# jinmang2/anomaly_detection_on_video

Hardware: AMD Instinct MI355X
Metric: 16-frame 224² RGB clips/sec (I3D extract→MIL score), 1/2/4/8 GPU + %MFMA-peak (higher is better)
Workload: dtype f32

## Files before the change

### anomaly_detection_on_video_amd/_lib.py

```python
from __future__ import annotations

import ctypes as C
import os
from typing import Optional

import torch

_HERE = os.path.dirname(os.path.abspath(__file__))
LIB_PATH = os.path.join(_HERE, "csrc", "libadvhip.so")

ALGO_AUTO = 0
ALGO_IGEMM_128x128 = 1
ALGO_IGEMM_128x64 = 2
ALGO_IGEMM_64x64 = 3
ALGO_IGEMM_64x128 = 4
ALGO_IGEMM_128x128x32 = 5
ALGO_IGEMM_128x64x32 = 6
ALGO_IGEMM_64x64x32 = 7
ALGO_IGEMM_64x128x32 = 8
ALGO_IGEMM_256x64 = 9
ALGO_FAST_BASE = 32
IGEMM_ALGOS = (1, 2, 3, 4, 5, 6, 7, 8)
FAST_ALGOS = tuple(ALGO_FAST_BASE + a for a in IGEMM_ALGOS)
ALGO_DMA_BASE = 64
DMA_ALGOS = tuple(ALGO_DMA_BASE + a for a in (1, 2, 3, 4, 6, 7, 8))
ALGO_DMA4_BASE = 96
DMA4_ALGOS = tuple(ALGO_DMA4_BASE + a for a in (2, 3, 4))
ALGO_BF16X3_BASE = 128
BF16X3_ALGOS = tuple(ALGO_BF16X3_BASE + a for a in (5, 6))
ALGO_DMA2_BASE = 160
DMA2_ALGOS = tuple(ALGO_DMA2_BASE + a for a in (1, 2, 3, 4, 6, 7, 8, 9))
ALGO_TSPAN_128x64 = 192
ALGO_MIXED_128x64 = 200
ALGO_PERSIST_BASE = 224
PERSIST_ALGOS = tuple(ALGO_PERSIST_BASE + t + 8 * (w - 1) for w in (1, 2, 3) for t in (2, 3))


def algo_tile(algo: int):
    if algo in (ALGO_TSPAN_128x64, ALGO_MIXED_128x64):
        return (128, 64, 16)
    if ALGO_PERSIST_BASE <= algo < ALGO_PERSIST_BASE + 32:
        return (128 if (algo - ALGO_PERSIST_BASE) & 7 == 2 else 64, 64, 16)
    if algo == ALGO_DMA2_BASE + ALGO_IGEMM_256x64:
        return (256, 64, 16)
    if algo >= ALGO_DMA2_BASE:
        algo -= ALGO_DMA2_BASE
    if algo >= ALGO_BF16X3_BASE:
        algo -= ALGO_BF16X3_BASE
    if algo >= ALGO_DMA4_BASE:
        algo -= ALGO_DMA4_BASE
    if algo >= ALGO_DMA_BASE:
        algo -= ALGO_DMA_BASE
    if algo >= ALGO_FAST_BASE:
        algo -= ALGO_FAST_BASE
    t = (algo - 1) & 3
    return (128 if t in (0, 1) else 64, 128 if t in (0, 3) else 64, 32 if algo >= 5 else 16)


class HipExtensionError(RuntimeError):
    pass


class ConvDesc(C.Structure):
    _fields_ = [(n, C.c_int32) for n in (
        "B", "Cin", "T", "H", "W", "Cout", "kt", "kh", "kw", "st", "sh", "sw", "pt", "ph", "pw",
        "relu", "algo", "splits")]


_P = C.c_void_p
_I = C.c_int32
_L = C.c_int64
# ... 2 lines not shown
class ConvEpilogue(C.Structure):
    _fields_ = ([(n, C.c_void_p) for n in ("y_preact", "dact_z", "ln_u", "ln_mu", "ln_rs", "splitk_counters")] + [("splitk_counter_bytes", C.c_int64)]
                + [("avgpool_out", C.c_void_p)])


class ColsumItem(C.Structure):
    _fields_ = [("src", C.c_void_p), ("dst", C.c_void_p), ("rows", C.c_int64), ("cols", C.c_int32), ("period", C.c_int32)]


class AdamItem(C.Structure):
    _fields_ = [(n, C.c_void_p) for n in ("param", "grad", "exp_avg", "exp_avg_sq", "step")] + [("n", C.c_int64)]


class NtItem(C.Structure):
    _fields_ = [(n, C.c_void_p) for n in ("A", "B", "C", "rowsum")] + [("M", C.c_int32), ("N", C.c_int32), ("lda", C.c_int64), ("ldb", C.c_int64)]


class GemmDesc(C.Structure):
    _fields_ = ([(n, C.c_int32) for n in ("M", "N", "K", "batch")]
                + [(n, C.c_int64) for n in ("sAb", "sAm", "sAk", "sBb", "sBk", "sBn", "sCb", "sCm", "sCn")]
                + [("alpha", C.c_float), ("beta", C.c_float), ("act", C.c_int32)]
                + [(n, C.c_void_p) for n in ("bias_m", "bias_n", "ln_u", "ln_mu", "ln_rs", "residual")])


SIGNATURES = {
    "advhip_abi_version": (C.c_int, []),
    "advhip_last_error": (C.c_char_p, []),
    "advhip_target_arch": (C.c_char_p, []),
    "advhip_conv3d_out_dims": (C.c_int, [C.POINTER(ConvDesc), C.POINTER(_I), C.POINTER(_I), C.POINTER(_I)]),
    "advhip_conv3d_packed_rows": (C.c_int, [C.POINTER(ConvDesc)]),
    "advhip_conv3d_pack_weight_f32": (C.c_int, [C.POINTER(ConvDesc), _P, _P, _P]),
    "advhip_conv3d_pack_weight_bf16x3": (C.c_int, [C.POINTER(ConvDesc), _P, _P, _P]),
    "advhip_conv3d_build_ktab": (C.c_int, [C.POINTER(ConvDesc), _P, _P]),
    "advhip_bn_fold_f32": (C.c_int, [_P, _P, _P, _P, C.c_float, _I, _P, _P, _P]),
    "advhip_conv3d_workspace_bytes": (_L, [C.POINTER(ConvDesc)]),
    "advhip_conv3d_bn_act_f32": (C.c_int, [C.POINTER(ConvDesc), _P, _P, _P, _P, _P, _P, _P, _P, _L, _P]),
    "advhip_conv3d_bn_act_strided_f32": (C.c_int, [C.POINTER(ConvDesc), _P, _L, _P, _P, _P, _P, _P, _P, _L, _P, _L, _P]),
    "advhip_conv3d_pool_out_dims": (C.c_int, [C.POINTER(ConvDesc)] + [_I] * 6 + [C.POINTER(_I)] * 3),
    "advhip_conv3d_relu_maxpool233_workspace_bytes": (_L, [C.POINTER(ConvDesc)]),
    "advhip_conv3d_bn_relu_maxpool233_f32": (C.c_int, [C.POINTER(ConvDesc), _P, _L, _P, _P, _P, _P, _P, _L, _P, _L, _P]),
    "advhip_split_w_plane_floats": (_I, [_I]),
    "advhip_split_w_f32": (C.c_int, [_P, _P, _L, _I, _P]),
    "advhip_conv3d_s2w_build_ktab": (C.c_int, [C.POINTER(ConvDesc), _P, _P]),
    "advhip_conv3d_s2w_bn_relu_maxpool233_f32": (C.c_int, [C.POINTER(ConvDesc), _P, _L, _P, _P, _P, _P, _P, _L, _P, _L, _P]),
    "advhip_conv3d_u8_table_sizes": (C.c_int, [C.POINTER(ConvDesc), C.POINTER(C.c_int64), C.POINTER(C.c_int64)]),
    "advhip_conv3d_u8_build_tables": (C.c_int, [C.POINTER(ConvDesc), _I, _I, _P, C.c_float, _P, _P, _P]),
    "advhip_conv3d_u8_taps_table_sizes": (C.c_int, [C.POINTER(ConvDesc), C.POINTER(C.c_int64), C.POINTER(C.c_int64), C.POINTER(C.c_int64)]),
    "advhip_conv3d_u8_taps_build_tables": (C.c_int, [C.POINTER(ConvDesc), _I, _I, _P, C.c_float, _P, _P, _P, _P]),
    "advhip_conv3d_u8_taps_tencrop_bn_relu_maxpool233_f32": (C.c_int, [C.POINTER(ConvDesc), _P, _L, _I, _I, _L, _L, _P, _P, _P, _P, _P,
                                                                       C.c_float, _P, _L, _P, _L, _P]),
    "advhip_conv3d_u8_tencrop_bn_relu_maxpool233_f32": (C.c_int, [C.POINTER(ConvDesc), _P, _L, _I, _I, _L, _P, _P, _P, _P, _P,
                                                                  C.c_float, _P, _L, _P, _L, _P]),
    "advhip_conv3d_u8_taps_tencrop_bn_relu_maxpool233_strided_f32": (C.c_int, [C.POINTER(ConvDesc), _P, _L, _I, _I, _I, _L, _L, _P, _P, _P, _P, _P,
                                                                               C.c_float, _P, _L, _P, _L, _P]),
    "advhip_conv3d_u8_tencrop_bn_relu_maxpool233_strided_f32": (C.c_int, [C.POINTER(ConvDesc), _P, _L, _I, _I, _I, _L, _P, _P, _P, _P, _P,
                                                                          C.c_float, _P, _L, _P, _L, _P]),
    "advhip_conv3d_bn_act_maxpool211_f32": (C.c_int, [C.POINTER(ConvDesc), _P, _L, _P, _P, _P, _P, _P, _P, _L, _P]),
    "advhip_bgemm_f32": (C.c_int, [C.POINTER(GemmDesc), _P, _P, _P, _P]),
    "advhip_gemm_nt_f32": (C.c_int, [_P, _P, _P, _I, _I, _I, _L, _L, _L, _I, _L, _P]),
    "advhip_gemm_nt_rowsum_f32": (C.c_int, [_P, _P, _P, _P, _I, _I, _I, _L, _L, _L, _I, _L, _I, _P]),
    "advhip_gemm_nt_workspace_bytes": (_L, [_I, _I, _I, _I]),
    "advhip_gemm_nt_reduced_f32": (C.c_int, [_P, _P, _P, _P, _I, _I, _I, _L, _L, _L, _I, _I, _P, _L, _P]),
    "advhip_gemm_nt_slabs_f32": (C.c_int, [_P, _P, _P, _I, _I, _I, _L, _L, _I, _I, _I, _P]),
    "advhip_sum_slabs_f32": (C.c_int, [_P, _P, _L, _I, _L, _P]),
    "advhip_gemm_nt_group_slabs_f32": (C.c_int, [C.POINTER(NtItem), _I, _I, _I, _L, _P]),
    "advhip_softmax_rows_f32": (C.c_int, [_P, _P, _L, _I, C.c_float, _P]),
# ... 132 lines not shown
```

### anomaly_detection_on_video_amd/csrc/conv_igemm.hip

```cpp
#include <algorithm>
#include <type_traits>
#include <utility>

#include "common.h"

namespace advhip {

struct FastDiv {
  unsigned mul, sh1, sh2, d;
  __host__ static FastDiv make(unsigned d) {
    FastDiv f;
    f.d = d;
    unsigned l = 0;
    while ((1ull << l) < d) ++l;
    f.mul = (unsigned)(((1ull << l) - d) * (1ull << 32) / d + 1);
    f.sh1 = l > 1 ? 1 : l;
    f.sh2 = l > 0 ? l - 1 : 0;
    if (l == 0) { f.mul = 0; f.sh1 = 0; f.sh2 = 0; }
    return f;
  }
  __device__ __forceinline__ unsigned div(unsigned n) const {
    const unsigned t = __umulhi(mul, n);
    return (t + ((n - t) >> sh1)) >> sh2;
  }
// ... 2600 lines not shown
};
static Geometry geometry(const advhip_conv3d_desc* d) {
  Geometry g;
  g.To = out_dim(d->T, d->kt, d->st, d->pt);
  g.Ho = out_dim(d->H, d->kh, d->sh, d->ph);
  g.Wo = out_dim(d->W, d->kw, d->sw, d->pw);
  g.M = (long long)d->B * g.To * g.Ho * g.Wo;
  g.K = d->Cin * d->kt * d->kh * d->kw;
  g.Kpad = (g.K + 31) / 32 * 32;
  return g;
}
}

namespace advhip {
static bool reduces_in_kernel(int algo) {
  return (algo >= ADVHIP_ALGO_DMA_BASE && algo < ADVHIP_ALGO_BF16X3_BASE) || algo >= ADVHIP_ALGO_DMA2_BASE;
}

static int device_cus() {
  static int cached[64] = {0};
  int dev = 0;
  if (hipGetDevice(&dev) != hipSuccess || dev < 0 || dev >= 64) return 256;
  if (cached[dev] == 0) {
    int n = 0;
    if (hipDeviceGetAttribute(&n, hipDeviceAttributeMultiprocessorCount, dev) != hipSuccess || n <= 0) n = 256;
    cached[dev] = n;
  }
  return cached[dev];
}
struct SplitLayout {
  int64_t cnt_bytes, part_bytes;
  int64_t total() const { return cnt_bytes + part_bytes; }
};
static SplitLayout split_layout(const advhip_conv3d_desc* d, const Geometry& g, const Choice& c) {
  if (c.splits <= 1) return {0, 0};
  if (!reduces_in_kernel(c.algo)) return {0, (int64_t)c.splits * g.M * d->Cout * (int64_t)sizeof(float)};
  int BM, BN, BK;
  tile_of(c.algo, &BM, &BN, &BK);
  const int64_t tiles = ((g.M + BM - 1) / BM) * (d->Cout / BN);
  return {(tiles * 4 + 255) / 256 * 256, tiles * c.splits * BM * BN * (int64_t)sizeof(float)};
}
}

namespace advhip {
static void set_bricks(ConvArgs& a, int nbt, int nbh, int nbw);

#ifndef ADVHIP_EXTRA_LDS
#define ADVHIP_EXTRA_LDS 0
#endif
template <int BM_, int BN_, int BK_>
static void launch_dma2(bool nocheck, bool s16, dim3 grid, hipStream_t st, const ConvArgs& a) {
  constexpr unsigned XL = ADVHIP_EXTRA_LDS;
  if (nocheck) {
    if (a.a16) hipLaunchKernelGGL((conv3d_igemm_dma_kernel<BM_, BN_, BK_, false, 2, EPI_STD, false, 2>), grid, dim3(256), XL, st, a);
    else hipLaunchKernelGGL((conv3d_igemm_dma_kernel<BM_, BN_, BK_, false, 2>), grid, dim3(256), XL, st, a);
    return;
  }
  if constexpr (BK_ == 16) {
    if (s16) {
      hipLaunchKernelGGL((conv3d_igemm_dma_kernel<BM_, BN_, BK_, true, 2, EPI_STD, false, 1>), grid, dim3(256), XL, st, a);
      return;
    }
  }
  hipLaunchKernelGGL((conv3d_igemm_dma_kernel<BM_, BN_, BK_, true, 2>), grid, dim3(256), XL, st, a);
}

}

extern "C" int64_t advhip_conv3d_workspace_bytes(const advhip_conv3d_desc* d) {
  if (validate(d)) return -1;
  const Geometry g = geometry(d);
  const Choice c = choose(d, g.M, g.Kpad);
  if (!instantiated(c.algo)) {
    set_error("conv3d: algo %d is not instantiated in this library", c.algo);
    return -1;
  }
  return split_layout(d, g, c).total();
}

extern "C" int advhip_conv3d_bn_act_f32(const advhip_conv3d_desc* d, const float* x, const float* w_packed,
                                        const int32_t* ktab, const float* scale, const float* shift,
                                        const float* residual, float* y, void* workspace, int64_t workspace_bytes,
                                        void* stream) {
  return advhip_conv3d_bn_act_strided_f32(d, x, 0, w_packed, ktab, scale, shift, residual, y, 0, workspace, workspace_bytes, stream);
}

extern "C" int advhip_conv3d_bn_act_strided_f32(const advhip_conv3d_desc* d, const float* x, int64_t x_batch_stride,
                                                const float* w_packed, const int32_t* ktab, const float* scale,
                                                const float* shift, const float* residual, float* y,
                                                int64_t y_batch_stride, void* workspace, int64_t workspace_bytes,
                                                void* stream) {
  return advhip_conv3d_bn_act_ex_f32(d, x, x_batch_stride, w_packed, ktab, scale, shift, residual, y, y_batch_stride, nullptr,
                                     workspace, workspace_bytes, stream);
}

extern "C" int advhip_conv3d_bn_act_ex_f32(const advhip_conv3d_desc* d, const float* x, int64_t x_batch_stride,
                                           const float* w_packed, const int32_t* ktab, const float* scale, const float* shift,
                                           const float* residual, float* y, int64_t y_batch_stride,
                                           const advhip_conv3d_epilogue* ep, void* workspace, int64_t workspace_bytes,
                                           void* stream) {
  if (int rc = validate(d)) return rc;
  float* y_preact = ep ? ep->y_preact : nullptr;
  const float* dact_z = ep ? ep->dact_z : nullptr;
  float* avg_out = ep ? ep->avgpool_out : nullptr;
  const bool ln = ep && ep->ln_u;
  ADVHIP_REQUIRE(!ep || (!ep->ln_u == !ep->ln_mu && !ep->ln_u == !ep->ln_rs), "conv3d: the LayerNorm fold needs ln_u, ln_mu and ln_rs together");
  ADVHIP_REQUIRE(d->relu >= 0 && d->relu <= ACT_MUL, "conv3d: unknown activation code %d (0 none, 1 ReLU, 2 GELU, 3 GELU + GELU' output, 4 multiplier)", d->relu);
  ADVHIP_REQUIRE(d->relu != ACT_GELU_D || (ep && ep->y_preact), "conv3d: activation code 3 writes GELU'(pre-activation) to the epilogue's second output: y_preact is null");
  ADVHIP_REQUIRE(d->relu != ACT_MUL || (ep && ep->dact_z && residual == nullptr), "conv3d: activation code 4 multiplies by the epilogue's dact_z tensor (no residual): it is null");
  ADVHIP_REQUIRE(x && w_packed && ktab && scale && shift && (y || avg_out), "conv3d: null pointer");
  const Geometry g = geometry(d);
  ConvArgs a;
  a.x = x; a.w = w_packed; a.ktab = reinterpret_cast<const int4*>(ktab);
  a.scale = scale; a.shift = shift; a.res = residual; a.y = y;
  a.y2 = y_preact; a.dact = dact_z;
  a.ln_u = ln ? ep->ln_u : nullptr; a.ln_mu = ln ? ep->ln_mu : nullptr; a.ln_rs = ln ? ep->ln_rs : nullptr;
  a.B = d->B; a.Cin = d->Cin; a.T = d->T; a.H = d->H; a.W = d->W; a.Cout = d->Cout;
  a.st = d->st; a.sh = d->sh; a.sw = d->sw; a.pt = d->pt; a.ph = d->ph; a.pw = d->pw;
  a.To = g.To; a.Ho = g.Ho; a.Wo = g.Wo;
  const long long x_dense = (long long)d->Cin * d->T * d->H * d->W, y_dense = (long long)d->Cout * g.To * g.Ho * g.Wo;
  const long long xbs = x_batch_stride > 0 ? x_batch_stride : x_dense, ybs = y_batch_stride > 0 ? y_batch_stride : y_dense;
  ADVHIP_REQUIRE(xbs >= x_dense && ybs >= y_dense, "conv3d: batch strides (%lld, %lld) smaller than one sample (%lld, %lld)", xbs, ybs, x_dense, y_dense);
  const long long in_elems = (long long)(d->B - 1) * xbs + x_dense;
  const long long M = g.M;
  if (in_elems >= (1ll << 31) || (long long)d->B * ybs >= (1ll << 32) || M * d->Cout >= (1ll << 32) || M >= (1ll << 31)) {
    set_error("conv3d: tensor too large for 32-bit indexing (in=%lld, out=%lld elements)", in_elems, M * d->Cout);
    return ADVHIP_ERANGE;
  }
  a.M = (int)M;
  a.x_bstride = (int)xbs;
  a.y_bstride = (int)ybs;
  a.Kpad = g.Kpad;
  a.HWo = a.Ho * a.Wo; a.THWo = a.To * a.HWo;
  a.HW = d->H * d->W; a.THW = d->T * a.HW;
// ... 14 lines not shown
  if (avg_out != nullptr) {
    ADVHIP_REQUIRE(d->kt == 1 && d->kh == 1 && d->kw == 1 && d->st == 1 && d->sh == 1 && d->sw == 1 && d->pt == 0 && d->ph == 0 && d->pw == 0 &&
                       g.K == g.Kpad && a.THWo <= 128 && d->Cout % 64 == 0 && ((uintptr_t)x & 15) == 0 && !ln && y_preact == nullptr && dact_z == nullptr && a.relu <= 1,
                   "conv3d: avgpool_out needs a 1x1x1 stride-1 conv on <= 128 positions per sample (%d), Cin %% 16 == 0, Cout %% 64 == 0, x 16-byte aligned, "
                   "no other epilogue operand, activation none or ReLU", a.THWo);
    c.algo = ADVHIP_ALGO_DMA2_BASE + ADVHIP_ALGO_IGEMM_128x64;
    c.splits = 1;
  }
  if (ybs != y_dense && !reduces_in_kernel(c.algo)) c.splits = 1;
  ADVHIP_REQUIRE(!ln || (d->kt == 1 && d->kh == 1 && d->kw == 1 && d->st == 1 && d->sh == 1 && d->sw == 1 && d->pt == 0 && d->ph == 0 && d->pw == 0),
                 "conv3d: the LayerNorm fold applies to 1x1x1 stride-1 convs (per-position statistics of the input)");
  ADVHIP_REQUIRE((y_preact == nullptr && dact_z == nullptr && !ln) || c.splits == 1 || reduces_in_kernel(c.algo),
                 "conv3d: pre-activation output / GELU-backward multiplier need a fused epilogue (algo %d with %d splits reduces in a second launch)", c.algo, c.splits);
  int BM, BN, BK;
  tile_of(c.algo, &BM, &BN, &BK);
  ADVHIP_REQUIRE(instantiated(c.algo), "conv3d: algo %d is not instantiated in this library", c.algo);
  const bool fast = c.algo >= ADVHIP_ALGO_FAST_BASE;
  if (fast) {
    ADVHIP_REQUIRE(fast_ok(d, in_elems, (long long)g.Kpad * d->Cout),
                   "conv3d: fast kernel needs kernel extents <= 10 and < 3.75 GiB operands (k=%d,%d,%d)", d->kt, d->kh, d->kw);
    a.kt_ = d->kt; a.kh_ = d->kh; a.kw_ = d->kw;
    a.pad_off = d->pt * d->H * d->W + d->ph * d->W + d->pw;
    a.x_bytes = (unsigned)((in_elems + a.pad_off) * 4);
    a.w_bytes = (unsigned)((long long)g.Kpad * d->Cout * 4);
  }
  ADVHIP_REQUIRE(d->Cout % BN == 0, "conv3d: Cout=%d not a multiple of the %d-wide N tile", d->Cout, BN);
  ADVHIP_REQUIRE(g.Kpad % BK == 0 || BK == 16, "conv3d: internal: Kpad");
  a.splits = c.splits;
  a.slab = M * d->Cout;
  const int nk = (g.Kpad + BK - 1) / BK;
  ADVHIP_REQUIRE(c.splits >= 1 && c.splits <= nk && c.splits <= 64, "conv3d: bad split count %d (k-tiles %d)", c.splits, nk);
  a.part = nullptr; a.cnt = nullptr; a.part_bytes = 0;
  a.mix_big = a.mix_small = a.mix_mbase = 0;
  const SplitLayout lay = split_layout(d, g, c);
  if (c.splits > 1) {
    ADVHIP_REQUIRE(workspace != nullptr && workspace_bytes >= lay.total(),
                   "conv3d: split-K needs a %lld-byte workspace (got %lld); query advhip_conv3d_workspace_bytes",
                   (long long)lay.total(), (long long)workspace_bytes);
    if (reduces_in_kernel(c.algo)) {
      ADVHIP_REQUIRE(lay.part_bytes < 0xF0000000ll && (uintptr_t)workspace % 16 == 0,
                     "conv3d: split-K partial tiles need a 16-byte aligned workspace below 3.75 GiB (%lld bytes)", (long long)lay.part_bytes);
      a.cnt = reinterpret_cast<unsigned*>(workspace);
      a.part = reinterpret_cast<float*>(reinterpret_cast<char*>(workspace) + lay.cnt_bytes);
      a.part_bytes = (unsigned)lay.part_bytes;
    } else {
      a.y = reinterpret_cast<float*>(workspace);
    }
  }
  const bool nocheck = d->kt == 1 && d->kh == 1 && d->kw == 1 && d->pt == 0 && d->ph == 0 && d->pw == 0 && g.K == g.Kpad;
  long long Mv = M;
  bool a16pad = false;
  if (nocheck && d->st == 1 && d->sh == 1 && d->sw == 1 && a.THW % 4 != 0 && ((uintptr_t)x & 15) == 0 && c.splits == 1 &&
      ((c.algo > ADVHIP_ALGO_DMA2_BASE && c.algo <= ADVHIP_ALGO_DMA2_BASE + ADVHIP_ALGO_IGEMM_256x64) || c.algo == ADVHIP_ALGO_MIXED_128x64 || is_persist(c.algo)) && !ln && y_preact == nullptr && dact_z == nullptr) {
    a.MP = (a.THWo + 3) / 4 * 4;
    Mv = (long long)d->B * a.MP;
    if (Mv < (1ll << 31)) {
      a16pad = true;
      a.M = (int)Mv;
      a.dTHWo = FastDiv::make((unsigned)a.MP);
    } else {
      a.MP = a.THWo;
      Mv = M;
    }
  }
  if (avg_out != nullptr) {
    a.MP = 128;
    Mv = (long long)d->B * a.MP;
    ADVHIP_REQUIRE(Mv < (1ll << 31), "conv3d: too many samples for the fused mean");
    a16pad = true;
    a.M = (int)Mv;
    a.dTHWo = FastDiv::make((unsigned)a.MP);
    a.avg_out = avg_out;
  }
  a.tiles_m = (int)((Mv + BM - 1) / BM);
  a.tiles_n = d->Cout / BN;
  a.dTilesN = FastDiv::make((unsigned)a.tiles_n);
  a.dSplits = FastDiv::make((unsigned)c.splits);
  int tspan_bt = 0;
  if (c.algo == ADVHIP_ALGO_TSPAN_128x64) {
    ADVHIP_REQUIRE(d->kh == 1 && d->kw == 1 && d->st == 1 && d->sh == 1 && d->sw == 1 && d->ph == 0 && d->pw == 0 && 2 * d->pt + 1 == d->kt,
                   "conv3d: ADVHIP_ALGO_TSPAN needs a (kt,1,1) stride-1 conv with padding kt/2 (k=%d,%d,%d)", d->kt, d->kh, d->kw);
    ADVHIP_REQUIRE(c.splits == 1 && g.To % 2 == 0 && y_preact == nullptr && dact_z == nullptr && !ln,
                   "conv3d: ADVHIP_ALGO_TSPAN runs unsplit on an even number of frames (T=%d, splits=%d) without the MGFN epilogue operands", g.To, c.splits);
    tspan_bt = g.To % 4 == 0 ? 4 : 2;
    a.H = 1; a.W = d->H * d->W; a.Ho = 1; a.Wo = a.HWo;
    a.kh_ = 1; a.kw_ = 1;
    set_bricks(a, g.To / tspan_bt, 1, (a.Wo + 128 / tspan_bt - 1) / (128 / tspan_bt));
    a.Tp = 0;
    a.ktab_s2w = reinterpret_cast<const int2*>(a.ktab + g.Kpad);
    a.s2w_rowp = a.W;
  }
  dim3 grid((unsigned)(a.tiles_m * a.tiles_n * c.splits));
  hipStream_t st = (hipStream_t)stream;
  if (a.cnt != nullptr) {
    const int64_t tiles = (int64_t)a.tiles_m * a.tiles_n;
// ... 691 lines not shown
```

### anomaly_detection_on_video_amd/ops.py

```python
from __future__ import annotations

import os

import ctypes as C
from dataclasses import dataclass, field
from typing import Dict, Optional, Sequence, Tuple

import torch

from . import _lib
from ._lib import ConvDesc, check, ptr, require_gpu, stream


def _triple(v) -> Tuple[int, int, int]:
    if isinstance(v, int):
        return (v, v, v)
    v = tuple(int(i) for i in v)
    assert len(v) == 3
    return v


def conv_out_dims(in_thw: Sequence[int], k: Sequence[int], s: Sequence[int], p: Sequence[int]) -> Tuple[int, int, int]:
    return tuple((n + 2 * pp - kk) // ss + 1 for n, kk, ss, pp in zip(in_thw, k, s, p))


@dataclass
class PackedConv:

    cout: int
    cin: int
    kernel: Tuple[int, int, int]
    stride: Tuple[int, int, int]
    padding: Tuple[int, int, int]
    w_packed: torch.Tensor
    scale: torch.Tensor
    shift: torch.Tensor
    ktabs: Dict[Tuple[int, int, int], torch.Tensor] = field(default_factory=dict)
    ktabs_s2w: Dict[Tuple[int, int, int], torch.Tensor] = field(default_factory=dict)
    algo: int = _lib.ALGO_AUTO
    name: str = ""
    splits: int = 0
    weight: Optional[torch.Tensor] = None
    w_split: Optional[torch.Tensor] = None
    choices: Dict[Tuple[int, int, int, int], Tuple[int, int]] = field(default_factory=dict)

    def key(self, B: int, T: int, H: int, W: int) -> str:
        return ",".join(str(v) for v in (self.cin, self.cout, *self.kernel, *self.stride, *self.padding, B, T, H, W))

    def desc(self, B: int, T: int, H: int, W: int, relu: bool, algo: Optional[int] = None,
             splits: Optional[int] = None) -> ConvDesc:
        kt, kh, kw = self.kernel
        st, sh, sw = self.stride
        pt, ph, pw = self.padding
        if algo is None and splits is None:
            ch = self.choices.get((B, T, H, W))
            if ch is None:
                from . import tuned

                ch = tuned.lookup(self.key(B, T, H, W), (self.algo, self.splits))
                if ARITH == "bf16x3":
                    ch = (_lib.ALGO_BF16X3_BASE + 6, 1)
                self.choices[(B, T, H, W)] = ch
            algo, splits = ch
        return ConvDesc(B, self.cin, T, H, W, self.cout, kt, kh, kw, st, sh, sw, pt, ph, pw, int(relu),
                        self.algo if algo is None else algo, self.splits if splits is None else splits)


def bn_fold(gamma, beta, mean, var, eps: float) -> Tuple[torch.Tensor, torch.Tensor]:
    require_gpu(gamma, beta, mean, var)
    lib = _lib.load()
    c = gamma.numel()
    scale = torch.empty(c, device=gamma.device, dtype=torch.float32)
    shift = torch.empty_like(scale)
    check(lib.advhip_bn_fold_f32(ptr(gamma), ptr(beta), ptr(mean), ptr(var), C.c_float(eps), c, ptr(scale), ptr(shift), stream()), "bn_fold")
    return scale, shift


def _packed_rows(d: ConvDesc) -> int:
    kpad = _lib.load().advhip_conv3d_packed_rows(C.byref(d))
    if kpad < 0:
        check(kpad, "conv3d_packed_rows")
    return kpad


def _build_ktab(pc: PackedConv, thw: Tuple[int, int, int]) -> torch.Tensor:
    d = pc.desc(1, *thw, relu=False)
    ktab = torch.empty((_packed_rows(d) * 6,), device=pc.w_packed.device, dtype=torch.int32)
    check(_lib.load().advhip_conv3d_build_ktab(C.byref(d), ptr(ktab), stream()), "build_ktab")
    return ktab


def split_weight(pc: PackedConv) -> torch.Tensor:
    if pc.w_split is None:
        kt, kh, kw = pc.kernel
        d = pc.desc(1, kt, kh, kw, relu=False, algo=0, splits=1)
        out = torch.empty((2, pc.cout, pc.w_packed.shape[0]), device=pc.weight.device, dtype=torch.int16)
        check(_lib.load().advhip_conv3d_pack_weight_bf16x3(C.byref(d), ptr(pc.weight), ptr(out), stream()), "pack_weight_bf16x3")
        pc.w_split = out
    return pc.w_split


def ensure_ktab(pc: PackedConv, thw: Tuple[int, int, int], batch: Optional[int] = None) -> torch.Tensor:
    ktab = pc.ktabs.get(thw)
    if ktab is None:
        ktab = pc.ktabs[thw] = _build_ktab(pc, thw)
    if batch is not None:
        d = pc.desc(batch, *thw, relu=False)
        if _lib.ALGO_BF16X3_BASE <= d.algo < _lib.ALGO_DMA2_BASE:
            split_weight(pc)
    return ktab


def pack_conv(weight: torch.Tensor, gamma, beta, mean, var, eps: float, stride, padding, name: str = "",
              algo: int = _lib.ALGO_AUTO) -> PackedConv:
    require_gpu(weight)
    weight = weight.detach().contiguous()
    cout, cin, kt, kh, kw = weight.shape
    scale, shift = bn_fold(gamma.detach(), beta.detach(), mean.detach(), var.detach(), eps)
    pc = PackedConv(cout, cin, (kt, kh, kw), _triple(stride), _triple(padding), weight, scale, shift, name=name, algo=algo)
    d = pc.desc(1, kt, kh, kw, relu=False)
    wp = torch.empty((_packed_rows(d), cout), device=weight.device, dtype=torch.float32)
    check(_lib.load().advhip_conv3d_pack_weight_f32(C.byref(d), ptr(weight), ptr(wp), stream()), "pack_weight")
    pc.w_packed = wp
    pc.weight = weight
    return pc


ARITH = os.environ.get("ADV_ARITH", "f32")

_WORKSPACES: Dict[Tuple[torch.device, int], torch.Tensor] = {}


def workspace(dev: torch.device, nbytes: int) -> Optional[torch.Tensor]:
    if nbytes <= 0:
        return None
    key = (dev, torch.cuda.current_stream(dev).cuda_stream)
    ws = _WORKSPACES.get(key)
    if ws is None or ws.numel() * 4 < nbytes:
        ws = _WORKSPACES[key] = torch.empty(((nbytes + 3) // 4,), device=dev, dtype=torch.float32)
    return ws


# ... 36 lines not shown
def batch_stride(t: torch.Tensor) -> int:
    n, c, t_, h, w = t.shape
    inner = (t_ * h * w, h * w, w, 1)
    for dim in range(1, 5):
        if t.shape[dim] > 1 and t.stride(dim) != inner[dim - 1]:
            raise ValueError(f"tensor {tuple(t.shape)} with strides {tuple(t.stride())} is not dense within a sample")
    return int(t.stride(0)) if n > 1 else c * inner[0]


def conv3d_bn_act(x: torch.Tensor, pc: PackedConv, relu: bool = True, residual: Optional[torch.Tensor] = None,
                  algo: Optional[int] = None, out: Optional[torch.Tensor] = None, splits: Optional[int] = None) -> torch.Tensor:
    require_gpu(x, out, contiguous=False)
    require_gpu(residual)
    if x.dim() != 5 or x.shape[1] != pc.cin:
        raise ValueError(f"{pc.name}: expected (B,{pc.cin},T,H,W), got {tuple(x.shape)}")
    B, _, T, H, W = x.shape
    to, ho, wo = conv_out_dims((T, H, W), pc.kernel, pc.stride, pc.padding)
    if min(to, ho, wo) <= 0:
        raise ValueError(f"{pc.name}: input {tuple(x.shape)} smaller than the kernel")
    y = out if out is not None else torch.empty((B, pc.cout, to, ho, wo), device=x.device, dtype=torch.float32)
    if tuple(y.shape) != (B, pc.cout, to, ho, wo) or y.dtype != torch.float32 or y.device != x.device:
        raise ValueError(f"{pc.name}: out {tuple(y.shape)} {y.dtype} on {y.device} != {(B, pc.cout, to, ho, wo)} float32 on {x.device}")
    if residual is not None and residual.shape != y.shape:
        raise ValueError(f"{pc.name}: residual {tuple(residual.shape)} != output {tuple(y.shape)}")
    ktab = ensure_ktab(pc, (T, H, W))
    if algo is not None and splits is None:
        splits = 1
    d = pc.desc(B, T, H, W, relu, algo, splits)
    lib = _lib.load()
    need = lib.advhip_conv3d_workspace_bytes(C.byref(d))
    if need < 0:
        check(int(need), f"conv3d_workspace_bytes[{pc.name}]")
    ws = workspace(x.device, need)
    w = pc.w_packed
    if _lib.ALGO_BF16X3_BASE <= d.algo < _lib.ALGO_DMA2_BASE:
        w = split_weight(pc)
    xbs, ybs = batch_stride(x), batch_stride(y)
    ep = None
    if need > 0:
        cnt = splitk_counters(x.device)
        ep = C.byref(_lib.ConvEpilogue(None, None, None, None, None, ptr(cnt), cnt.numel() * 4))
    check(lib.advhip_conv3d_bn_act_ex_f32(C.byref(d), ptr(x), xbs, ptr(w), ptr(ktab), ptr(pc.scale), ptr(pc.shift), ptr(residual), ptr(y), ybs,
                                          ep, ptr(ws), need, stream()), f"conv3d[{pc.name}]")
    return y


def conv_pool_out_dims(in_thw: Sequence[int], pc: "PackedConv", pool_kernel, pool_stride) -> Tuple[int, int, int]:
    return conv_out_dims(conv_out_dims(in_thw, pc.kernel, pc.stride, pc.padding), _triple(pool_kernel), _triple(pool_stride), (0, 0, 0))


STEM_S2W = os.environ.get("ADV_STEM_S2W", "1") == "1"


def s2w_ok(pc: PackedConv, W: int) -> bool:
    kw, sw, pw = pc.kernel[2], pc.stride[2], pc.padding[2]
    return sw == 2 and kw % 2 == 1 and pw == kw // 2 and pw <= 4 and W % 8 == 0 and W >= 8 and pc.kernel[0] <= 10 and pc.kernel[1] <= 10


def split_w(x: torch.Tensor) -> torch.Tensor:
    require_gpu(x)
    B, Cc, T, H, W = x.shape
    lib = _lib.load()
    wp = lib.advhip_split_w_plane_floats(W)
    if wp < 0:
        raise ValueError(f"split_w: W = {W} must be even")
    xs = torch.empty((B, Cc, T, H, 2, wp), device=x.device, dtype=torch.float32)
    check(lib.advhip_split_w_f32(ptr(x), ptr(xs), B * Cc * T * H, W, stream(x)), "split_w")
    return xs


def ensure_ktab_s2w(pc: PackedConv, thw: Tuple[int, int, int]) -> torch.Tensor:
    tab = pc.ktabs_s2w.get(thw)
    if tab is None:
        d = pc.desc(1, *thw, relu=True, algo=0, splits=1)
        tab = torch.empty((_packed_rows(d) * 2,), device=pc.w_packed.device, dtype=torch.int32)
# ... 419 lines not shown
```

### include/advhip.h

```cpp
#ifndef ADVHIP_H
#define ADVHIP_H

#include <stddef.h>
#include <stdint.h>

#ifdef __cplusplus
extern "C" {
#endif

#define ADVHIP_ABI_VERSION 2

#define ADVHIP_OK 0
#define ADVHIP_EINVAL (-1)
#define ADVHIP_ELAUNCH (-2)
#define ADVHIP_ERANGE (-3)

#define ADVHIP_ALGO_AUTO 0
#define ADVHIP_ALGO_IGEMM_128x128 1
#define ADVHIP_ALGO_IGEMM_128x64 2
#define ADVHIP_ALGO_IGEMM_64x64 3
#define ADVHIP_ALGO_IGEMM_64x128 4
#define ADVHIP_ALGO_IGEMM_128x128x32 5
#define ADVHIP_ALGO_IGEMM_128x64x32 6
#define ADVHIP_ALGO_IGEMM_64x64x32 7
#define ADVHIP_ALGO_IGEMM_64x128x32 8
#define ADVHIP_ALGO_IGEMM_256x64 9
#define ADVHIP_ALGO_FAST_BASE 32
#define ADVHIP_ALGO_DMA_BASE 64
#define ADVHIP_ALGO_DMA4_BASE 96
#define ADVHIP_ALGO_BF16X3_BASE 128
#define ADVHIP_ALGO_DMA2_BASE 160
#define ADVHIP_ALGO_TSPAN_128x64 192
#define ADVHIP_ALGO_MIXED_128x64 200
#define ADVHIP_ALGO_PERSIST_BASE 224

typedef struct advhip_conv3d_desc {
  int32_t B, Cin, T, H, W;
  int32_t Cout, kt, kh, kw;
  int32_t st, sh, sw;
  int32_t pt, ph, pw;
  int32_t relu;
  int32_t algo;
  int32_t splits;
} advhip_conv3d_desc;

int advhip_abi_version(void);
const char* advhip_last_error(void);
const char* advhip_target_arch(void);

int advhip_conv3d_out_dims(const advhip_conv3d_desc* d, int32_t* To, int32_t* Ho, int32_t* Wo);

int advhip_conv3d_packed_rows(const advhip_conv3d_desc* d);

int advhip_conv3d_pack_weight_f32(const advhip_conv3d_desc* d, const float* w, float* w_packed,
                                  void* stream);

int advhip_conv3d_pack_weight_bf16x3(const advhip_conv3d_desc* d, const float* w, void* w_split, void* stream);

int advhip_conv3d_build_ktab(const advhip_conv3d_desc* d, int32_t* ktab, void* stream);

int advhip_bn_fold_f32(const float* gamma, const float* beta, const float* mean, const float* var,
                       float eps, int32_t C, float* scale, float* shift, void* stream);

int64_t advhip_conv3d_workspace_bytes(const advhip_conv3d_desc* d);
int advhip_conv3d_bn_act_f32(const advhip_conv3d_desc* d, const float* x, const float* w_packed,
                             const int32_t* ktab, const float* scale, const float* shift,
                             const float* residual, float* y, void* workspace,
                             int64_t workspace_bytes, void* stream);

int advhip_conv3d_bn_act_strided_f32(const advhip_conv3d_desc* d, const float* x, int64_t x_batch_stride,
                                     const float* w_packed, const int32_t* ktab, const float* scale, const float* shift,
                                     const float* residual, float* y, int64_t y_batch_stride, void* workspace,
                                     int64_t workspace_bytes, void* stream);

typedef struct advhip_conv3d_epilogue {
  float* y_preact;
  const float* dact_z;
  const float* ln_u;
  const float* ln_mu;
  const float* ln_rs;
  void* splitk_counters;
  int64_t splitk_counter_bytes;
  float* avgpool_out;
} advhip_conv3d_epilogue;
int advhip_conv3d_bn_act_ex_f32(const advhip_conv3d_desc* d, const float* x, int64_t x_batch_stride, const float* w_packed,
                                const int32_t* ktab, const float* scale, const float* shift, const float* residual, float* y,
                                int64_t y_batch_stride, const advhip_conv3d_epilogue* ep, void* workspace,
                                int64_t workspace_bytes, void* stream);

int advhip_chan_stats_f32(const float* x, float* mu, float* rs, int32_t C, int64_t N, float eps, void* stream);

int advhip_conv3d_pool_out_dims(const advhip_conv3d_desc* d, int32_t pkt, int32_t pkh, int32_t pkw, int32_t pst,
                                int32_t psh, int32_t psw, int32_t* Tp, int32_t* Hp, int32_t* Wp);

int64_t advhip_conv3d_relu_maxpool233_workspace_bytes(const advhip_conv3d_desc* d);
int advhip_conv3d_bn_relu_maxpool233_f32(const advhip_conv3d_desc* d, const float* x, int64_t x_batch_stride,
                                         const float* w_packed, const int32_t* ktab, const float* scale, const float* shift,
                                         float* y, int64_t y_batch_stride, void* workspace, int64_t workspace_bytes,
                                         void* stream);

int32_t advhip_split_w_plane_floats(int32_t W);
int advhip_split_w_f32(const float* x, float* xs, int64_t rows, int32_t W, void* stream);
int advhip_conv3d_s2w_build_ktab(const advhip_conv3d_desc* d, int32_t* ktab_s2w, void* stream);
int advhip_conv3d_s2w_bn_relu_maxpool233_f32(const advhip_conv3d_desc* d, const float* xs, int64_t xs_batch_stride,
                                             const float* w_packed, const int32_t* ktab_s2w, const float* scale, const float* shift,
                                             float* y, int64_t y_batch_stride, void* workspace, int64_t workspace_bytes,
                                             void* stream);

int advhip_tencrop_normalize_planes_u8(const uint8_t* frames, float* xs, int32_t F, int32_t H, int32_t W, int32_t C,
                                       int32_t frames_per_clip, int32_t crop, int64_t first_crop_clip, int64_t count, float mean,
                                       float stdv, void* stream);
int advhip_tencrop_normalize_planes_u8_strided(const uint8_t* frames, float* xs, int32_t F, int32_t H, int32_t W, int32_t C,
                                               int32_t frames_per_clip, int32_t clip_stride, int32_t crop, int64_t first_crop_clip,
                                               int64_t count, float mean, float stdv, void* stream);

int advhip_conv3d_u8_table_sizes(const advhip_conv3d_desc* d, int64_t* ktab_ints, int64_t* corr_floats);
int advhip_conv3d_u8_build_tables(const advhip_conv3d_desc* d, int32_t FH, int32_t FW, const float* w_packed, float mean,
                                  int32_t* ktab_u8, float* corr, void* stream);
int advhip_conv3d_u8_tencrop_bn_relu_maxpool233_f32(const advhip_conv3d_desc* d, const uint8_t* frames, int64_t F, int32_t FH,
                                                    int32_t FW, int64_t first_crop_clip, const float* w_packed,
                                                    const int32_t* ktab_u8, const float* corr,
// ... 235 lines not shown
```

Baseline: 3871.

## Add temporal-fold conv algo mapping short-T (kt,1,1) convs onto pointwise GEMM

After: 4066, median of 6. 5.0% higher.

```diff
diff --git a/anomaly_detection_on_video_amd/_lib.py b/anomaly_detection_on_video_amd/_lib.py
--- a/anomaly_detection_on_video_amd/_lib.py
+++ b/anomaly_detection_on_video_amd/_lib.py
@@ -32,11 +32,19 @@
 DMA2_ALGOS = tuple(ALGO_DMA2_BASE + a for a in (1, 2, 3, 4, 6, 7, 8, 9))
 ALGO_TSPAN_128x64 = 192
 ALGO_MIXED_128x64 = 200
+ALGO_TFOLD_BASE = 208
+TFOLD_ALGOS = tuple(ALGO_TFOLD_BASE + a for a in (1, 2, 3, 4, 6, 7, 8, 9))
 ALGO_PERSIST_BASE = 224
 PERSIST_ALGOS = tuple(ALGO_PERSIST_BASE + t + 8 * (w - 1) for w in (1, 2, 3) for t in (2, 3))
 
 
+def is_tfold(algo: int) -> bool:
+    return ALGO_TFOLD_BASE <= algo < ALGO_TFOLD_BASE + 16
+
+
 def algo_tile(algo: int):
+    if is_tfold(algo):
+        algo += ALGO_DMA2_BASE - ALGO_TFOLD_BASE
     if algo in (ALGO_TSPAN_128x64, ALGO_MIXED_128x64):
         return (128, 64, 16)
     if ALGO_PERSIST_BASE <= algo < ALGO_PERSIST_BASE + 32:
@@ -105,6 +113,9 @@
     "advhip_conv3d_pack_weight_f32": (C.c_int, [C.POINTER(ConvDesc), _P, _P, _P]),
     "advhip_conv3d_pack_weight_bf16x3": (C.c_int, [C.POINTER(ConvDesc), _P, _P, _P]),
     "advhip_conv3d_build_ktab": (C.c_int, [C.POINTER(ConvDesc), _P, _P]),
+    "advhip_conv3d_tfold_desc": (C.c_int, [C.POINTER(ConvDesc), C.POINTER(ConvDesc)]),
+    "advhip_conv3d_pack_weight_tfold_f32": (C.c_int, [C.POINTER(ConvDesc), _P, _P, _P]),
+    "advhip_conv3d_tfold_scale_shift_f32": (C.c_int, [C.POINTER(ConvDesc), _P, _P, _P, _P, _P]),
     "advhip_bn_fold_f32": (C.c_int, [_P, _P, _P, _P, C.c_float, _I, _P, _P, _P]),
     "advhip_conv3d_workspace_bytes": (_L, [C.POINTER(ConvDesc)]),
     "advhip_conv3d_bn_act_f32": (C.c_int, [C.POINTER(ConvDesc), _P, _P, _P, _P, _P, _P, _P, _P, _L, _P]),
diff --git a/anomaly_detection_on_video_amd/csrc/conv_igemm.hip b/anomaly_detection_on_video_amd/csrc/conv_igemm.hip
--- a/anomaly_detection_on_video_amd/csrc/conv_igemm.hip
+++ b/anomaly_detection_on_video_amd/csrc/conv_igemm.hip
@@ -2656,14 +2656,28 @@
   int64_t cnt_bytes, part_bytes;
   int64_t total() const { return cnt_bytes + part_bytes; }
 };
-static SplitLayout split_layout(const advhip_conv3d_desc* d, const Geometry& g, const Choice& c) {
+static SplitLayout split_layout(const advhip_conv3d_desc* d, const Geometry& g, const Choice& c, long long Mv) {
   if (c.splits <= 1) return {0, 0};
   if (!reduces_in_kernel(c.algo)) return {0, (int64_t)c.splits * g.M * d->Cout * (int64_t)sizeof(float)};
   int BM, BN, BK;
   tile_of(c.algo, &BM, &BN, &BK);
-  const int64_t tiles = ((g.M + BM - 1) / BM) * (d->Cout / BN);
+  const int64_t tiles = ((Mv + BM - 1) / BM) * (d->Cout / BN);
   return {(tiles * 4 + 255) / 256 * 256, tiles * c.splits * BM * BN * (int64_t)sizeof(float)};
 }
+
+static bool is_nocheck(const advhip_conv3d_desc* d, const Geometry& g) {
+  return d->kt == 1 && d->kh == 1 && d->kw == 1 && d->pt == 0 && d->ph == 0 && d->pw == 0 && g.K == g.Kpad;
+}
+
+static long long padded_rows(const advhip_conv3d_desc* d, const Geometry& g, const Choice& c) {
+  const long long thw = (long long)g.To * g.Ho * g.Wo;
+  if (!(is_nocheck(d, g) && d->st == 1 && d->sh == 1 && d->sw == 1 && thw % 4 != 0)) return 0;
+  if (!((c.algo > ADVHIP_ALGO_DMA2_BASE && c.algo <= ADVHIP_ALGO_DMA2_BASE + ADVHIP_ALGO_IGEMM_256x64) || c.algo == ADVHIP_ALGO_MIXED_128x64 || is_persist(c.algo))) return 0;
+  const long long Mv = (long long)d->B * ((thw + 3) / 4 * 4);
+  return Mv < (1ll << 31) ? Mv : 0;
+}
+
+static bool is_tfold(int algo) { return algo >= ADVHIP_ALGO_TFOLD_BASE && algo < ADVHIP_ALGO_TFOLD_BASE + 16; }
 }
 
 namespace advhip {
@@ -2693,13 +2707,18 @@
 
 extern "C" int64_t advhip_conv3d_workspace_bytes(const advhip_conv3d_desc* d) {
   if (validate(d)) return -1;
+  if (is_tfold(d->algo)) {
+    advhip_conv3d_desc f;
+    return advhip_conv3d_tfold_desc(d, &f) ? -1 : advhip_conv3d_workspace_bytes(&f);
+  }
   const Geometry g = geometry(d);
   const Choice c = choose(d, g.M, g.Kpad);
   if (!instantiated(c.algo)) {
     set_error("conv3d: algo %d is not instantiated in this library", c.algo);
     return -1;
   }
-  return split_layout(d, g, c).total();
+  const long long Mp = padded_rows(d, g, c);
+  return split_layout(d, g, c, Mp > g.M ? Mp : g.M).total();
 }
 
 extern "C" int advhip_conv3d_bn_act_f32(const advhip_conv3d_desc* d, const float* x, const float* w_packed,
@@ -2724,6 +2743,14 @@
                                            const advhip_conv3d_epilogue* ep, void* workspace, int64_t workspace_bytes,
                                            void* stream) {
   if (int rc = validate(d)) return rc;
+  if (is_tfold(d->algo)) {
+    advhip_conv3d_desc f;
+    if (int rc = advhip_conv3d_tfold_desc(d, &f)) return rc;
+    ADVHIP_REQUIRE(!ep || (ep->ln_u == nullptr && ep->avgpool_out == nullptr),
+                   "conv3d: ADVHIP_ALGO_TFOLD takes neither the LayerNorm fold nor avgpool_out (both are per position of the unfolded conv)");
+    return advhip_conv3d_bn_act_ex_f32(&f, x, x_batch_stride, w_packed, ktab, scale, shift, residual, y, y_batch_stride, ep, workspace,
+                                       workspace_bytes, stream);
+  }
   float* y_preact = ep ? ep->y_preact : nullptr;
   const float* dact_z = ep ? ep->dact_z : nullptr;
   float* avg_out = ep ? ep->avgpool_out : nullptr;
@@ -2804,7 +2831,17 @@
   ADVHIP_REQUIRE(c.splits >= 1 && c.splits <= nk && c.splits <= 64, "conv3d: bad split count %d (k-tiles %d)", c.splits, nk);
   a.part = nullptr; a.cnt = nullptr; a.part_bytes = 0;
   a.mix_big = a.mix_small = a.mix_mbase = 0;
-  const SplitLayout lay = split_layout(d, g, c);
+  const bool nocheck = is_nocheck(d, g);
+  long long Mv = M;
+  bool a16pad = false;
+  if (const long long Mp = padded_rows(d, g, c); Mp > 0 && ((uintptr_t)x & 15) == 0 && !ln && y_preact == nullptr && dact_z == nullptr) {
+    a.MP = (a.THWo + 3) / 4 * 4;
+    Mv = Mp;
+    a16pad = true;
+    a.M = (int)Mv;
+    a.dTHWo = FastDiv::make((unsigned)a.MP);
+  }
+  const SplitLayout lay = split_layout(d, g, c, Mv);
   if (c.splits > 1) {
     ADVHIP_REQUIRE(workspace != nullptr && workspace_bytes >= lay.total(),
                    "conv3d: split-K needs a %lld-byte workspace (got %lld); query advhip_conv3d_workspace_bytes",
@@ -2817,22 +2854,6 @@
       a.part_bytes = (unsigned)lay.part_bytes;
     } else {
       a.y = reinterpret_cast<float*>(workspace);
-    }
-  }
-  const bool nocheck = d->kt == 1 && d->kh == 1 && d->kw == 1 && d->pt == 0 && d->ph == 0 && d->pw == 0 && g.K == g.Kpad;
-  long long Mv = M;
-  bool a16pad = false;
-  if (nocheck && d->st == 1 && d->sh == 1 && d->sw == 1 && a.THW % 4 != 0 && ((uintptr_t)x & 15) == 0 && c.splits == 1 &&
-      ((c.algo > ADVHIP_ALGO_DMA2_BASE && c.algo <= ADVHIP_ALGO_DMA2_BASE + ADVHIP_ALGO_IGEMM_256x64) || c.algo == ADVHIP_ALGO_MIXED_128x64 || is_persist(c.algo)) && !ln && y_preact == nullptr && dact_z == nullptr) {
-    a.MP = (a.THWo + 3) / 4 * 4;
-    Mv = (long long)d->B * a.MP;
-    if (Mv < (1ll << 31)) {
-      a16pad = true;
-      a.M = (int)Mv;
-      a.dTHWo = FastDiv::make((unsigned)a.MP);
-    } else {
-      a.MP = a.THWo;
-      Mv = M;
     }
   }
   if (avg_out != nullptr) {
diff --git a/anomaly_detection_on_video_amd/csrc/conv_tfold.hip b/anomaly_detection_on_video_amd/csrc/conv_tfold.hip
--- /dev/null
+++ b/anomaly_detection_on_video_amd/csrc/conv_tfold.hip
@@ -0,0 +1,84 @@
+#include <algorithm>
+
+#include "common.h"
+
+namespace advhip {
+
+__global__ void pack_weight_tfold_kernel(const float* __restrict__ w, float* __restrict__ wf, int Cin, int kt, int pt, int T, int K,
+                                         int Kpad, int N) {
+  const long long total = (long long)Kpad * N;
+  for (long long i = (long long)blockIdx.x * blockDim.x + threadIdx.x; i < total; i += (long long)gridDim.x * blockDim.x) {
+    const int k = (int)(i / N), n2 = (int)(i - (long long)k * N);
+    float v = 0.f;
+    if (k < K) {
+      const int ci = k / T, ti = k - ci * T;
+      const int n = n2 / T, t = n2 - n * T;
+      const int dt = ti - t + pt;
+      v = w[((long long)n * Cin + ci) * kt + dt];
+    }
+    wf[i] = v;
+  }
+}
+
+__global__ void expand_scale_shift_tfold_kernel(const float* __restrict__ scale, const float* __restrict__ shift,
+                                                float* __restrict__ scale_f, float* __restrict__ shift_f, int T, int N) {
+  const int i = blockIdx.x * blockDim.x + threadIdx.x;
+  if (i < N) {
+    scale_f[i] = scale[i / T];
+    shift_f[i] = shift[i / T];
+  }
+}
+
+}
+
+using namespace advhip;
+
+extern "C" int advhip_conv3d_tfold_desc(const advhip_conv3d_desc* d, advhip_conv3d_desc* folded) {
+  if (int rc = advhip_conv3d_out_dims(d, nullptr, nullptr, nullptr)) return rc;
+  ADVHIP_REQUIRE(folded != nullptr, "conv3d: ADVHIP_ALGO_TFOLD: null folded descriptor");
+  ADVHIP_REQUIRE(d->kh == 1 && d->kw == 1 && d->ph == 0 && d->pw == 0,
+                 "conv3d: ADVHIP_ALGO_TFOLD is not instantiated for this conv: it needs a (kt,1,1) conv without spatial padding (k=%d,%d,%d, p=%d,%d,%d)", d->kt, d->kh, d->kw, d->pt,
+                 d->ph, d->pw);
+  ADVHIP_REQUIRE(d->st == 1 && d->sh == 1 && d->sw == 1, "conv3d: ADVHIP_ALGO_TFOLD is not instantiated for this conv: it needs stride 1 (s=%d,%d,%d)", d->st, d->sh, d->sw);
+  ADVHIP_REQUIRE(2 * d->pt + 1 == d->kt, "conv3d: ADVHIP_ALGO_TFOLD is not instantiated for this conv: it needs the centred padding pt = kt/2 of an odd kt (kt=%d, pt=%d)", d->kt, d->pt);
+  ADVHIP_REQUIRE(d->T <= d->pt + 1, "conv3d: ADVHIP_ALGO_TFOLD is not instantiated for this conv: it needs T <= pt + 1 frames, one tap per (output, input) frame pair (T=%d, pt=%d)",
+                 d->T, d->pt);
+  ADVHIP_REQUIRE((long long)d->Cin * d->T < (1ll << 31) && (long long)d->Cout * d->T < (1ll << 31), "conv3d: ADVHIP_ALGO_TFOLD: folded channels overflow");
+  int algo = d->algo;
+  if (algo >= ADVHIP_ALGO_TFOLD_BASE && algo < ADVHIP_ALGO_TFOLD_BASE + 16) {
+    const int tile = algo - ADVHIP_ALGO_TFOLD_BASE;
+    ADVHIP_REQUIRE(tile >= 1 && tile <= 9 && tile != 5, "conv3d: algo %d is not instantiated in this library (ADVHIP_ALGO_TFOLD_BASE + tile id 1..4, 6..9 of the 2-deep LDS-DMA family)", d->algo);
+    algo = ADVHIP_ALGO_DMA2_BASE + tile;
+  }
+  advhip_conv3d_desc f = *d;
+  f.Cin = d->Cin * d->T;
+  f.Cout = d->Cout * d->T;
+  f.T = 1;
+  f.kt = 1;
+  f.pt = 0;
+  f.algo = algo;
+  *folded = f;
+  return ADVHIP_OK;
+}
+
+extern "C" int advhip_conv3d_pack_weight_tfold_f32(const advhip_conv3d_desc* d, const float* w, float* w_folded, void* stream) {
+  advhip_conv3d_desc f;
+  if (int rc = advhip_conv3d_tfold_desc(d, &f)) return rc;
+  ADVHIP_REQUIRE(w && w_folded, "pack_weight_tfold: null pointer");
+  const int K = f.Cin, Kpad = advhip_conv3d_packed_rows(&f);
+  if (Kpad < 0) return Kpad;
+  const long long total = (long long)Kpad * f.Cout;
+  const int grid = (int)std::min<long long>((total + 255) / 256, 256 * 16);
+  hipLaunchKernelGGL(pack_weight_tfold_kernel, dim3(grid), dim3(256), 0, (hipStream_t)stream, w, w_folded, d->Cin, d->kt, d->pt, d->T, K, Kpad, f.Cout);
+  return check_launch("pack_weight_tfold");
+}
+
+extern "C" int advhip_conv3d_tfold_scale_shift_f32(const advhip_conv3d_desc* d, const float* scale, const float* shift, float* scale_folded,
+                                                   float* shift_folded, void* stream) {
+  advhip_conv3d_desc f;
+  if (int rc = advhip_conv3d_tfold_desc(d, &f)) return rc;
+  ADVHIP_REQUIRE(scale && shift && scale_folded && shift_folded, "tfold_scale_shift: null pointer");
+  hipLaunchKernelGGL(expand_scale_shift_tfold_kernel, dim3((f.Cout + 255) / 256), dim3(256), 0, (hipStream_t)stream, scale, shift, scale_folded,
+                     shift_folded, d->T, f.Cout);
+  return check_launch("tfold_scale_shift");
+}
diff --git a/anomaly_detection_on_video_amd/ops.py b/anomaly_detection_on_video_amd/ops.py
--- a/anomaly_detection_on_video_amd/ops.py
+++ b/anomaly_detection_on_video_amd/ops.py
@@ -42,6 +42,8 @@
     splits: int = 0
     weight: Optional[torch.Tensor] = None
     w_split: Optional[torch.Tensor] = None
+    tfold_w: Dict[int, Tuple[torch.Tensor, torch.Tensor, torch.Tensor]] = field(default_factory=dict)
+    tfold_ktabs: Dict[Tuple[int, int, int], torch.Tensor] = field(default_factory=dict)
     choices: Dict[Tuple[int, int, int, int], Tuple[int, int]] = field(default_factory=dict)
 
     def key(self, B: int, T: int, H: int, W: int) -> str:
@@ -100,6 +102,37 @@
     return pc.w_split
 
 
+def tfold_desc(d: ConvDesc) -> ConvDesc:
+    f = ConvDesc()
+    check(_lib.load().advhip_conv3d_tfold_desc(C.byref(d), C.byref(f)), "conv3d_tfold_desc")
+    return f
+
+
+def tfold_operands(pc: PackedConv, thw: Tuple[int, int, int]) -> Tuple[torch.Tensor, torch.Tensor, torch.Tensor, torch.Tensor]:
+    T = thw[0]
+    d = pc.desc(1, *thw, relu=False, algo=0, splits=1)
+    ops_t = pc.tfold_w.get(T)
+    ktab = pc.tfold_ktabs.get(thw)
+    if ops_t is not None and ktab is not None:
+        return ops_t[0], ktab, ops_t[1], ops_t[2]
+    if pc.weight is None:
+        raise _lib.HipExtensionError(f"{pc.name}: the temporal fold packs its operand from the torch-layout weights, which this conv does not keep")
+    f = tfold_desc(d)
+    lib = _lib.load()
+    dev = pc.w_packed.device
+    if ops_t is None:
+        wf = torch.empty((_packed_rows(f), f.Cout), device=dev, dtype=torch.float32)
+        check(lib.advhip_conv3d_pack_weight_tfold_f32(C.byref(d), ptr(pc.weight), ptr(wf), stream()), f"pack_weight_tfold[{pc.name}]")
+        sc, sh = torch.empty((f.Cout,), device=dev, dtype=torch.float32), torch.empty((f.Cout,), device=dev, dtype=torch.float32)
+        check(lib.advhip_conv3d_tfold_scale_shift_f32(C.byref(d), ptr(pc.scale), ptr(pc.shift), ptr(sc), ptr(sh), stream()), f"tfold_scale_shift[{pc.name}]")
+        ops_t = pc.tfold_w[T] = (wf, sc, sh)
+    if ktab is None:
+        ktab = torch.empty((_packed_rows(f) * 6,), device=dev, dtype=torch.int32)
+        check(lib.advhip_conv3d_build_ktab(C.byref(f), ptr(ktab), stream()), f"build_ktab_tfold[{pc.name}]")
+        pc.tfold_ktabs[thw] = ktab
+    return ops_t[0], ktab, ops_t[1], ops_t[2]
+
+
 def ensure_ktab(pc: PackedConv, thw: Tuple[int, int, int], batch: Optional[int] = None) -> torch.Tensor:
     ktab = pc.ktabs.get(thw)
     if ktab is None:
@@ -108,6 +141,8 @@
         d = pc.desc(batch, *thw, relu=False)
         if _lib.ALGO_BF16X3_BASE <= d.algo < _lib.ALGO_DMA2_BASE:
             split_weight(pc)
+        if _lib.is_tfold(d.algo):
+            tfold_operands(pc, thw)
     return ktab
 
 
@@ -210,15 +245,17 @@
     if need < 0:
         check(int(need), f"conv3d_workspace_bytes[{pc.name}]")
     ws = workspace(x.device, need)
-    w = pc.w_packed
+    w, scale, shift = pc.w_packed, pc.scale, pc.shift
     if _lib.ALGO_BF16X3_BASE <= d.algo < _lib.ALGO_DMA2_BASE:
         w = split_weight(pc)
+    if _lib.is_tfold(d.algo):
+        w, ktab, scale, shift = tfold_operands(pc, (T, H, W))
     xbs, ybs = batch_stride(x), batch_stride(y)
     ep = None
     if need > 0:
         cnt = splitk_counters(x.device)
         ep = C.byref(_lib.ConvEpilogue(None, None, None, None, None, ptr(cnt), cnt.numel() * 4))
-    check(lib.advhip_conv3d_bn_act_ex_f32(C.byref(d), ptr(x), xbs, ptr(w), ptr(ktab), ptr(pc.scale), ptr(pc.shift), ptr(residual), ptr(y), ybs,
+    check(lib.advhip_conv3d_bn_act_ex_f32(C.byref(d), ptr(x), xbs, ptr(w), ptr(ktab), ptr(scale), ptr(shift), ptr(residual), ptr(y), ybs,
                                           ep, ptr(ws), need, stream()), f"conv3d[{pc.name}]")
     return y
 
diff --git a/include/advhip.h b/include/advhip.h
--- a/include/advhip.h
+++ b/include/advhip.h
@@ -32,6 +32,7 @@
 #define ADVHIP_ALGO_DMA2_BASE 160
 #define ADVHIP_ALGO_TSPAN_128x64 192
 #define ADVHIP_ALGO_MIXED_128x64 200
+#define ADVHIP_ALGO_TFOLD_BASE 208
 #define ADVHIP_ALGO_PERSIST_BASE 224
 
 typedef struct advhip_conv3d_desc {
@@ -87,6 +88,11 @@
                                 const int32_t* ktab, const float* scale, const float* shift, const float* residual, float* y,
                                 int64_t y_batch_stride, const advhip_conv3d_epilogue* ep, void* workspace,
                                 int64_t workspace_bytes, void* stream);
+
+int advhip_conv3d_tfold_desc(const advhip_conv3d_desc* d, advhip_conv3d_desc* folded);
+int advhip_conv3d_pack_weight_tfold_f32(const advhip_conv3d_desc* d, const float* w, float* w_folded, void* stream);
+int advhip_conv3d_tfold_scale_shift_f32(const advhip_conv3d_desc* d, const float* scale, const float* shift, float* scale_folded,
+                                        float* shift_folded, void* stream);
 
 int advhip_chan_stats_f32(const float* x, float* mu, float* rs, int32_t C, int64_t N, float eps, void* stream);
 
```
